# WeGoToMars/indexed_bzip2

Measured on AMD Instinct MI355X. Metric: decompressed MB/s (whole node), 2 GiB Silesia bz2-9, higher is better.
Workload: dtype u8

## Files before the change

### indexed_bzip2_amd/csrc/bz2_device.hip

```cpp
#include <hip/hip_runtime.h>

#include <cstdio>
#include <atomic>
#include <chrono>
#include <cstdlib>
#include <algorithm>
#include <cstring>
#include <condition_variable>
#include <map>
#include <memory>
#include <mutex>
#include <string>
#include <thread>
#include <vector>

#include "../../include/mi355x_bz2.h"
#include "bz2_kernels.hip.h"
#include "bz2_lines.hip.h"
#include "bz2_stage1.hip.h"
#include "bz2_hscan.hip.h"
#include "bz2_walk.hip.h"
#include "bz2_plan.hpp"
#include "bz2_scratch.hpp"
#include "bz2_lanes.hpp"
// ... 271 lines not shown
    if ( buffer.copyIssued ) {
        HIP_TRY( c, hipStreamWaitEvent( c->stream, buffer.copied, 0 ) );
    }
    if ( size + 256 > buffer.capacity ) {
        HIP_TRY( c, hipStreamSynchronize( c->stream ) );
        if ( buffer.copyIssued ) HIP_TRY( c, hipEventSynchronize( buffer.copied ) );
        HIP_TRY( c, buffer.grow( c, size + 256, size + size / 8 + ( 1u << 20 ), size ) );
    }
    buffer.copyIssued = false;
    c->outCurrent = target;
    c->dOut = buffer.bytes;
    return MI355X_BZ2_OK;
}

const char* const KERNEL_NAMES[] = {
    "(k_huff: gone)", "k_mtf<272>", "k_bwt_build", "k_walk", "k_link2", "k_emit", "k_replicate", "k_rle<false>",
    "k_rle<true>", "k_crc", "k_walk_plan", "k_mtf<144>", "k_hscan", "k_hsym"
};
constexpr uint32_t N_KERNELS = sizeof( KERNEL_NAMES ) / sizeof( KERNEL_NAMES[0] );
static_assert( N_KERNELS <= MI355X_BZ2_MAX_KERNELS );
}

struct WalkChain
{
    std::mutex mutex;
    hipEvent_t events[64]{};
    uint32_t next{ 0 };
    hipEvent_t last{ nullptr };
    std::atomic<int> liveContexts{ 0 };
};
WalkChain g_walkChains[16];
WalkChain& walkChainOf( int device ) { return g_walkChains[(unsigned)device % 16u]; }
// ... 56 lines not shown
        return v != nullptr && v[0] == '1';
    };
    BatchSwitches s;
    s.plan.scanWaves = positive( "MI355X_BZ2_SCAN_WAVES" );
    s.plan.bwtSplit = positive( "MI355X_BZ2_BWT_SPLIT" );
    s.plan.mtfNarrow = one( "MI355X_BZ2_MTF_NARROW" );
    s.plan.noSplit = one( "MI355X_BZ2_NO_SPLIT" );
    s.trace = one( "MI355X_BZ2_TRACE" );
    s.readerTrace = std::getenv( "MI355X_BZ2_READER_TRACE" ) != nullptr;
    return s;
}

int
queueOutput( mi355x_bz2_ctx* c, uint32_t n, const uint64_t* overflow )
{
    TIMED_LAUNCH( c, 0, c->stream, 8, k_rle<true>, dim3( n ), dim3( RLE_THREADS ), 0, c->stream, c->dMeta, c->dR, c->dOut,
                  overflow );
    TIMED_LAUNCH( c, 0, c->stream, 9, k_crc, dim3( n ), dim3( CRC_THREADS ), 0, c->stream, c->dMeta, c->dOut, c->crc,
                  overflow );
    HIP_TRY( c, hipEventRecord( c->evStep[2], c->stream ) );
    HIP_TRY( c, hipGetLastError() );
    HIP_TRY( c, hipMemcpyAsync( c->hMeta, c->dMeta, (size_t)n * sizeof( BlockMeta ), hipMemcpyDeviceToHost, c->stream ) );
    return MI355X_BZ2_OK;
}

int
ensureLanes( mi355x_bz2_ctx* c, const LaneLayout& layout )
{
    for ( uint32_t l = 1; l < layout.lanes; ++l ) {
        if ( (int)l == layout.highLane ) {
            if ( c->highStream == nullptr ) {
                int leastPriority = 0, greatestPriority = 0;
                (void)hipDeviceGetStreamPriorityRange( &leastPriority, &greatestPriority );
                HIP_TRY( c, hipStreamCreateWithPriority( &c->highStream, hipStreamNonBlocking, greatestPriority ) );
// ... 606 lines not shown
            const std::scoped_lock walkLock( walks.mutex );
            if ( walks.last != nullptr ) HIP_TRY( c, hipStreamWaitEvent( q, walks.last, 0 ) );
            TIMED_LAUNCH( c, g, q, 3, k_walk, walkGrid, dim3( WALK_THREADS ), 0, q,
                          meta, tab, walkPlan, walkBlk, walkPre, segLen, segSucc, plan.walkChunk, stash, segCont );
            hipEvent_t& slot = walks.events[walks.next++ % 64];
            if ( slot == nullptr ) HIP_TRY( c, hipEventCreateWithFlags( &slot, hipEventDisableTiming ) );
            HIP_TRY( c, hipEventRecord( slot, q ) );
            walks.last = slot;
        }
        TIMED_LAUNCH( c, g, q, 4, k_link2, dim3( m ), dim3( LINK_THREADS ), sizeof( LinkShared ), q, meta, segLen, segSucc, chain );
        TIMED_LAUNCH( c, g, q, 5, k_emit, dim3( ( SEG_STRIDE + EMIT_THREADS * EMIT_TILES - 1 ) / ( EMIT_THREADS * EMIT_TILES ), m ), dim3( EMIT_THREADS ), 0, q,
                      meta, tab, chain, stash, segCont, rbuf );
        static_assert( (size_t)SEG_STRIDE * STASH_BYTES >= L_STRIDE );
        TIMED_LAUNCH( c, g, q, 6, k_replicate, dim3( m ), dim3( 256 ), 0, q, meta, rbuf, reinterpret_cast<uint8_t*>( stash ),
                      (size_t)SEG_STRIDE * STASH_BYTES );
        TIMED_LAUNCH( c, g, q, 7, k_rle<false>, dim3( m ), dim3( RLE_THREADS ), 0, q, meta, rbuf, (uint8_t*)nullptr );
        lastGroupOfLane[layout.laneOf[g]] = g;
    }
    HIP_TRY( c, hipGetLastError() );
    for ( uint32_t l = 1; l < MAX_LANES; ++l ) {
        const int g = lastGroupOfLane[l];
        if ( g < 0 ) continue;
        HIP_TRY( c, hipEventRecord( c->evGroupDone[g], streamOfLane( (int)l ) ) );
        HIP_TRY( c, hipStreamWaitEvent( c->stream, c->evGroupDone[g], 0 ) );
    }

    if ( c->outputHold != nullptr ) {
        HIP_TRY( c, hipStreamWaitEvent( c->stream, c->outputHold, 0 ) );
        c->outputHold = nullptr;
    }
    hipLaunchKernelGGL( k_offsets, dim3( 1 ), dim3( OFFSETS_THREADS ), 0, c->stream, c->dMeta, c->dSlotOf, n,
                        c->out[c->outCurrent].capacity, c->dTotals );
    rc = queueOutput( c, n, c->dTotals + 1 );
    if ( rc != MI355X_BZ2_OK ) return rc;
    HIP_TRY( c, hipMemcpyAsync( c->hTotals, c->dTotals, 2 * sizeof( uint64_t ), hipMemcpyDeviceToHost, c->stream ) );
    c->pendingBlocks = n;
    if ( switches.readerTrace ) {
        const auto ms = [] ( auto a, auto b ) { return std::chrono::duration<double, std::milli>( b - a ).count(); };
        std::fprintf( stderr, "[device] begin of %u blocks: scratch %.1f ms, input %.1f ms, plan + launches %.1f ms\n", n,
                      ms( tBegin, tScratch ), ms( tScratch, tInput ), ms( tInput, std::chrono::steady_clock::now() ) );
    }
    return MI355X_BZ2_OK;
}

int
mi355x::resultBuffer( mi355x_bz2_ctx* c, uint64_t size, uint64_t keep, uint8_t** device )
{
// ... 592 lines not shown
```

### indexed_bzip2_amd/csrc/bz2_kernels.hip.h

```cpp
#pragma once

#include <hip/hip_runtime.h>
#include <stdint.h>

#include "bz2_scratch.hpp"

namespace bz2gpu
{
constexpr uint32_t MAX_N = 900000;
constexpr uint32_t MIN_SEG_STRIDE = 16;
constexpr uint32_t MARK = 0x80000000u;
constexpr uint32_t LF_MASK = 0xFFFFFu;
constexpr uint32_t INVALID_OFF = 0xFFFFFFFFu;

enum Status : int32_t {
    ST_OK = 0, ST_EOF = 1, ST_BAD_MAGIC = 2, ST_RANDOMIZED = 3, ST_ORIGPTR_RANGE = 4, ST_GROUP_COUNT = 5,
    ST_SELECTOR_COUNT = 6, ST_SELECTOR_UNARY = 7, ST_CODE_LENGTH = 8, ST_HUFFMAN_LENGTHS = 9,
    ST_SELECTOR_OVERRUN = 10, ST_INVALID_CODE = 11, ST_RUN_OVERFLOW = 12, ST_DATA_OVERFLOW = 13,
    ST_ORIGPTR_DATA = 14, ST_CRC = 15
};

struct BlockMeta
{
    uint64_t enc_off;
// ... 400 lines not shown
            R[N - 1 - k] = R[N - 1 - ( k % c )];
        }
        return;
    }
    uint8_t* const Y = tmp_buf + (size_t)b * tmp_stride;
    for ( uint32_t k = threadIdx.x; k < c; k += 256 ) Y[k] = R[N - 1 - k];
    __syncthreads();
    for ( uint32_t k = threadIdx.x; k < N; k += 256 ) {
        R[N - 1 - k] = Y[( k % c + c - r ) % c];
    }
}

constexpr uint32_t RLE_THREADS = 512;
constexpr uint32_t RLE_BYTES_PER_THREAD = 32;
constexpr uint32_t RLE_TILE = RLE_THREADS * RLE_BYTES_PER_THREAD;
constexpr uint32_t FN_IDENTITY = 0 | ( 1 << 3 ) | ( 2 << 6 ) | ( 3 << 9 ) | ( 4 << 12 );

__device__ __forceinline__ uint32_t
fn_apply( uint32_t f, uint32_t k )
{
    return ( f >> ( 3 * k ) ) & 7u;
}

__device__ __forceinline__ uint32_t
fn_compose( uint32_t f, uint32_t g )
{
    uint32_t h = 0;
#pragma unroll
    for ( int k = 0; k < 5; ++k ) h |= fn_apply( g, fn_apply( f, k ) ) << ( 3 * k );
    return h;
}

__device__ __forceinline__ uint32_t
rle_step( uint32_t k, bool eq )
{
    return eq ? ( k == 4 ? 0u : k + 1 ) : ( k == 4 ? 0u : 1u );
}

constexpr uint32_t OFFSETS_THREADS = 1024;

__global__ __launch_bounds__( OFFSETS_THREADS ) void
k_offsets( BlockMeta* meta, const uint32_t* __restrict__ slot_of, uint32_t n, uint64_t capacity, uint64_t* result )
{
    __shared__ uint64_t partial[OFFSETS_THREADS];
    const uint32_t t = threadIdx.x;
    const uint32_t per = ( n + OFFSETS_THREADS - 1 ) / OFFSETS_THREADS;
    const uint32_t lo = t * per < n ? t * per : n;
    const uint32_t hi = lo + per < n ? lo + per : n;
    uint64_t sum = 0;
    for ( uint32_t i = lo; i < hi; ++i ) {
        const BlockMeta& m = meta[slot_of[i]];
        sum += m.walk_ok ? m.decoded_size : 0;
    }
    partial[t] = sum;
    __syncthreads();
    for ( uint32_t step = 1; step < OFFSETS_THREADS; step *= 2 ) {
        const uint64_t add = t >= step ? partial[t - step] : 0;
        __syncthreads();
        partial[t] += add;
        __syncthreads();
    }
    uint64_t off = partial[t] - sum;
    for ( uint32_t i = lo; i < hi; ++i ) {
        BlockMeta& m = meta[slot_of[i]];
        m.out_off = off;
        off += m.walk_ok ? m.decoded_size : 0;
    }
    if ( t == OFFSETS_THREADS - 1 ) {
        result[0] = partial[t];
        result[1] = partial[t] + 256 > capacity ? 1 : 0;
    }
}

template<bool WRITE>
__global__ __launch_bounds__( RLE_THREADS ) void
k_rle( BlockMeta*                   meta,
       const uint8_t* __restrict__  r_buf,
       uint8_t* __restrict__        out,
       const uint64_t*              skip = nullptr )
{
    __shared__ uint32_t wfn[RLE_THREADS / 64];
    __shared__ uint64_t wsum[RLE_THREADS / 64];
    __shared__ uint32_t carryFn;
    __shared__ uint64_t carrySum;
    __shared__ uint16_t fnTab[256];
    __shared__ uint16_t cmTab[5][256];
    const uint32_t b = blockIdx.x;
    const BlockMeta mt = meta[b];
    if ( !mt.walk_ok ) return;
    if ( WRITE && skip != nullptr && *skip != 0 ) return;
    if ( threadIdx.x < 256 ) {
        const uint32_t e = threadIdx.x;
        uint32_t t[5] = { 0, 1, 2, 3, 4 };
        for ( uint32_t q = 0; q < 8; ++q ) {
            const bool eq = ( e >> q ) & 1u;
            for ( uint32_t k = 0; k < 5; ++k ) t[k] = rle_step( t[k], eq );
        }
        fnTab[e] = (uint16_t)( t[0] | ( t[1] << 3 ) | ( t[2] << 6 ) | ( t[3] << 9 ) | ( t[4] << 12 ) );
        for ( uint32_t k = 0; k < 5; ++k ) {
            uint32_t state = k, counts = 0;
            for ( uint32_t q = 0; q < 8; ++q ) {
                if ( state == 4 ) counts |= 1u << q;
                state = rle_step( state, ( e >> q ) & 1u );
            }
            cmTab[k][e] = (uint16_t)( counts | ( state << 8 ) );
        }
    }
    __syncthreads();
    const uint32_t N = mt.n;
    const uint8_t* const R = r_buf + (size_t)b * L_STRIDE;
    uint8_t* const dst = WRITE ? out + mt.out_off : nullptr;
    const uint32_t tid = threadIdx.x, wave = tid >> 6, lane = tid & 63;

    uint32_t stateIn = 0;
    uint64_t sumIn = 0;

    for ( uint32_t tile = 0; tile < N; tile += RLE_TILE ) {
        const uint32_t i0 = tile + tid * RLE_BYTES_PER_THREAD;
        uint32_t wv[RLE_BYTES_PER_THREAD / 4] = {};
        uint32_t prev = 0;
        uint32_t nb = 0;
        if ( i0 < N ) {
            nb = N - i0 < RLE_BYTES_PER_THREAD ? N - i0 : RLE_BYTES_PER_THREAD;
            const uint4 v = *reinterpret_cast<const uint4*>( R + i0 );
            const uint4 v2 = *reinterpret_cast<const uint4*>( R + i0 + 16 );
            wv[0] = v.x; wv[1] = v.y; wv[2] = v.z; wv[3] = v.w;
            wv[4] = v2.x; wv[5] = v2.y; wv[6] = v2.z; wv[7] = v2.w;
            prev = i0 > 0 ? R[i0 - 1] : 0x100u;
        }
        uint32_t eqMask = 0;
        const bool full = nb == RLE_BYTES_PER_THREAD;
        if ( full ) {
            uint32_t before = prev << 24;
#pragma unroll
            for ( uint32_t j = 0; j < RLE_BYTES_PER_THREAD / 4; ++j ) {
                const uint32_t d = wv[j] ^ __builtin_amdgcn_alignbit( wv[j], before, 24 );
                const uint32_t nonZero = ( ( ( d & 0x7F7F7F7Fu ) + 0x7F7F7F7Fu ) | d ) & 0x80808080u;
                const uint32_t e = ( ~nonZero >> 7 ) & 0x01010101u;
                eqMask |= ( ( e * 0x01020408u ) >> 24 & 0xFu ) << ( 4 * j );
                before = wv[j];
            }
            if ( prev > 0xFFu ) eqMask &= ~1u;
        } else {
            uint32_t p = prev;
            _Pragma( "unroll" ) for ( uint32_t q = 0; q < RLE_BYTES_PER_THREAD; ++q ) { if ( q >= nb ) break;
                const uint32_t c = ( wv[q >> 2] >> ( 8 * ( q & 3 ) ) ) & 0xFFu;
                eqMask |= ( c == p ? 1u : 0u ) << q;
                p = c;
            }
        }
        uint32_t fn = FN_IDENTITY;
        if ( full ) {
            fn = fn_compose( fn_compose( fnTab[eqMask & 0xFFu], fnTab[( eqMask >> 8 ) & 0xFFu] ),
                             fn_compose( fnTab[( eqMask >> 16 ) & 0xFFu], fnTab[eqMask >> 24] ) );
        } else if ( nb > 0 ) {
            uint32_t t0 = 0, t1 = 1, t2 = 2, t3 = 3, t4 = 4;
            _Pragma( "unroll" ) for ( uint32_t q = 0; q < RLE_BYTES_PER_THREAD; ++q ) { if ( q >= nb ) break;
                const bool eq = ( eqMask >> q ) & 1u;
                t0 = rle_step( t0, eq ); t1 = rle_step( t1, eq ); t2 = rle_step( t2, eq );
                t3 = rle_step( t3, eq ); t4 = rle_step( t4, eq );
            }
            fn = t0 | ( t1 << 3 ) | ( t2 << 6 ) | ( t3 << 9 ) | ( t4 << 12 );
        }
        uint32_t incl = fn;
        for ( int d = 1; d < 64; d <<= 1 ) {
            const uint32_t o = __shfl_up( incl, d );
            if ( (int)lane >= d ) incl = fn_compose( o, incl );
        }
        if ( lane == 63 ) wfn[wave] = incl;
        __syncthreads();
        uint32_t pre = FN_IDENTITY;
        for ( uint32_t w = 0; w < wave; ++w ) pre = fn_compose( pre, wfn[w] );
        uint32_t exclWave = __shfl_up( incl, 1 );
        if ( lane == 0 ) exclWave = FN_IDENTITY;
        const uint32_t before = fn_compose( pre, exclWave );
        uint32_t k = fn_apply( before, stateIn );

        uint32_t mySize = 0;
        uint32_t countMask = 0;
        if ( full ) {
            uint32_t r = cmTab[k][eqMask & 0xFFu];
            countMask = r & 0xFFu;
            r = cmTab[r >> 8][( eqMask >> 8 ) & 0xFFu];
            countMask |= ( r & 0xFFu ) << 8;
            r = cmTab[r >> 8][( eqMask >> 16 ) & 0xFFu];
            countMask |= ( r & 0xFFu ) << 16;
            r = cmTab[r >> 8][eqMask >> 24];
            countMask |= ( r & 0xFFu ) << 24;
            mySize = RLE_BYTES_PER_THREAD - (uint32_t)__popc( countMask );
            if ( countMask != 0 ) {
#pragma unroll
                for ( uint32_t j = 0; j < RLE_BYTES_PER_THREAD / 4; ++j ) {
                    const uint32_t four = ( countMask >> ( 4 * j ) ) & 0xFu;
                    if ( four != 0 ) {
#pragma unroll
                        for ( uint32_t z = 0; z < 4; ++z ) {
                            if ( ( four >> z ) & 1u ) mySize += ( wv[j] >> ( 8 * z ) ) & 0xFFu;
                        }
                    }
                }
            }
        } else {
            uint32_t kk = k;
            _Pragma( "unroll" ) for ( uint32_t q = 0; q < RLE_BYTES_PER_THREAD; ++q ) { if ( q >= nb ) break;
                const uint32_t c = ( wv[q >> 2] >> ( 8 * ( q & 3 ) ) ) & 0xFFu;
                if ( kk == 4 ) { mySize += c; countMask |= 1u << q; } else { mySize += 1; }
                kk = rle_step( kk, ( eqMask >> q ) & 1u );
            }
        }
        uint32_t inclS = mySize;
        for ( int d = 1; d < 64; d <<= 1 ) {
            const uint32_t o = __shfl_up( inclS, d );
            if ( (int)lane >= d ) inclS += o;
        }
        if ( lane == 63 ) wsum[wave] = inclS;
        __syncthreads();
        uint64_t preS = 0, tileTotal = 0;
        for ( uint32_t w = 0; w < RLE_THREADS / 64; ++w ) {
            if ( w < wave ) preS += wsum[w];
            tileTotal += wsum[w];
        }
        const uint64_t myOff = sumIn + preS + ( inclS - mySize );

        if constexpr ( WRITE ) {
            if ( countMask == 0 && nb == RLE_BYTES_PER_THREAD ) {
                uint8_t* const d = dst + myOff;
                const uint32_t head = ( 4u - ( (uint32_t)myOff & 3u ) ) & 3u;
                for ( uint32_t z = 0; z < head; ++z ) d[z] = (uint8_t)( wv[0] >> ( 8 * z ) );
                uint32_t* const d32 = reinterpret_cast<uint32_t*>( d + head );
#pragma unroll
                for ( uint32_t j = 0; j + 1 < RLE_BYTES_PER_THREAD / 4; ++j ) {
                    d32[j] = __builtin_amdgcn_alignbyte( wv[j + 1], wv[j], head );
                }
                constexpr uint32_t LAST = RLE_BYTES_PER_THREAD / 4 - 1;
                if ( head == 0 ) {
                    d32[LAST] = wv[LAST];
                } else {
                    for ( uint32_t z = head; z < 4; ++z ) d[4 * LAST + z] = (uint8_t)( wv[LAST] >> ( 8 * z ) );
                }
            } else {
            uint64_t o = myOff;
            uint32_t p = prev;
            _Pragma( "unroll" ) for ( uint32_t q = 0; q < RLE_BYTES_PER_THREAD; ++q ) { if ( q >= nb ) break;
                const uint32_t c = ( wv[q >> 2] >> ( 8 * ( q & 3 ) ) ) & 0xFFu;
                if ( ( countMask >> q ) & 1u ) {
                    for ( uint32_t z = 0; z < c; ++z ) dst[o + z] = (uint8_t)p;
                    o += c;
                } else {
                    dst[o++] = (uint8_t)c;
                }
                p = c;
            }
            }
        }

        if ( tid == RLE_THREADS - 1 ) {
            carryFn = fn_apply( fn_compose( before, fn ), stateIn );
        }
        __syncthreads();
        stateIn = carryFn;
        sumIn += tileTotal;
        __syncthreads();
    }
    if ( !WRITE && tid == 0 ) {
        meta[b].decoded_size = sumIn;
    }
    (void)carrySum;
}

constexpr uint32_t CRC_THREADS = 256;
constexpr uint32_t CRC_CHUNK_LOG2 = 8;
constexpr uint32_t CRC_CHUNK = 1u << CRC_CHUNK_LOG2;
constexpr uint32_t CRC_TILE = CRC_THREADS * CRC_CHUNK;
constexpr uint32_t CRC_POLY = 0x04C11DB7u;

__device__ __forceinline__ uint32_t
gf_mul( uint32_t a, uint32_t b )
{
    uint32_t r = 0;
#pragma unroll 8
    for ( int i = 31; i >= 0; --i ) {
        r = ( r << 1 ) ^ ( ( r >> 31 ) ? CRC_POLY : 0u );
        if ( ( a >> i ) & 1u ) r ^= b;
    }
    return r;
}

__device__ __forceinline__ uint32_t
gf_pow8( const uint32_t* table, uint64_t nbytes )
{
    uint32_t r = 0x00000001u;
    for ( int k = 0; nbytes != 0 && k < 32; ++k, nbytes >>= 1 ) {
        if ( nbytes & 1u ) r = gf_mul( r, table[k] );
    }
    return r;
}

__global__ __launch_bounds__( CRC_THREADS ) void
k_crc( BlockMeta*                  meta,
       const uint8_t* __restrict__ out,
       CrcConsts                   cc,
       const uint64_t*             skip = nullptr )
{
    __shared__ uint32_t table[256];
    __shared__ uint32_t wcrc[CRC_THREADS / 64];
    const uint32_t b = blockIdx.x;
// ... 56 lines not shown
            running = gf_mul( running, cc.pow8[CRC_CHUNK_LOG2 + 8] ) ^ tileCrc;
        }
        __syncthreads();
        tEnd = t + CRC_TILE;
    }
    if ( tid == 0 ) {
        const uint64_t pad = tEnd - a1;
        uint32_t pure = D == 0 ? 0u : gf_mul( running, gf_pow8( cc.ipow8, pad ) );
        const uint32_t init = gf_mul( 0xFFFFFFFFu, gf_pow8( cc.pow8, D ) );
        const uint32_t crc = ~( pure ^ init );
        meta[b].computed_crc = crc;
        if ( crc != mt.header_crc ) meta[b].status = ST_CRC;
    }
}

constexpr uint32_t GATHER_THREADS = 256;
constexpr uint64_t GATHER_TILE = 32768;

struct GatherTile
{
    uint64_t src, dst, size;
};

__global__ __launch_bounds__( GATHER_THREADS ) void
k_gather( const GatherTile* __restrict__ tiles, const uint8_t* __restrict__ src, uint8_t* __restrict__ dst )
{
    const GatherTile t = tiles[blockIdx.x];
    const uint8_t* const s = src + t.src;
    uint8_t* const d = dst + t.dst;
    const uint32_t n = (uint32_t)t.size;
// ... 32 lines not shown
```

### indexed_bzip2_amd/csrc/bz2_scratch.hpp

```cpp
#pragma once

#include <algorithm>
#include <cstdint>

#include "bz2_plan.hpp"

namespace bz2gpu
{
constexpr uint32_t L_STRIDE = 900096;
constexpr uint32_t SEL_STRIDE = 32768;
constexpr uint32_t TAB_STRIDE = 1u << 20;
constexpr uint32_t KMAX = 32768;
constexpr uint32_t SEG_STRIDE = KMAX + 64;
constexpr uint32_t STASH_BYTES = 128;
constexpr uint32_t SYM_STRIDE = SEG_STRIDE * 64;
constexpr uint32_t GPOS_STRIDE = 18048;
constexpr int BWT_WAVES = 16;
constexpr uint32_t BWT_COUNTS_PER_BLOCK = BWT_SPLIT_MAX * BWT_WAVES * 256;

struct ScratchSizes
{
    uint64_t blockMeta, huffMeta, scanMeta, huffTables, walkPlan;
};

enum ScratchMemory : bool { DEVICE = false, PINNED = true };

#define BZ2_SCRATCH_REGIONS( X )                                                                                              \
    X( DEVICE, dOffsets, uint64_t, n * sizeof( uint64_t ), OWN )                                                              \
    X( DEVICE, dOrder, uint32_t, n * sizeof( uint32_t ), OWN )                                                                \
    X( DEVICE, dMeta, BlockMeta, n * s.blockMeta, OWN )                                                                       \
    X( DEVICE, dSel, uint8_t, n * SEL_STRIDE + 256, OWN )                                                                     \
    X( DEVICE, dStb, uint8_t, n * 256, OWN )                                                                                  \
    X( DEVICE, dHmeta, HuffMeta, n * s.huffMeta, OWN )                                                                        \
    X( DEVICE, dSmeta, ScanMeta, n * s.scanMeta, OWN )                                                 \
    X( DEVICE, dHtab, HuffTables, n * s.huffTables, OWN )                                        \
    X( DEVICE, dGpos, uint32_t, n * GPOS_STRIDE * sizeof( uint32_t ), OWN )                                                   \
    X( DEVICE, dL, uint8_t, n * L_STRIDE + 256, OWN )                                                                         \
    X( DEVICE, dTab, uint32_t, n * TAB_STRIDE * sizeof( uint32_t ), OWN )                                                     \
        \
    X( DEVICE, dR, uint8_t, n * L_STRIDE + 256, keepStages ? OWN : R_dL )                                                     \
    X( DEVICE, dSegLen, uint32_t, n * SEG_STRIDE * sizeof( uint32_t ), OWN )                                                  \
    X( DEVICE, dSegSucc, uint32_t, n * SEG_STRIDE * sizeof( uint32_t ), OWN )                                                 \
    X( DEVICE, dSegCont, uint32_t, n * SEG_STRIDE * sizeof( uint32_t ), OWN )  \
    X( DEVICE, dChain, uint2, n * SEG_STRIDE * 2 * sizeof( uint32_t ), OWN )  \
    X( DEVICE, dStash, uint32_t, n * SEG_STRIDE * STASH_BYTES, OWN )                        \
        \
    X( DEVICE, dSym, uint16_t, n * SYM_STRIDE * sizeof( uint16_t ), R_dStash )                                                \
    X( DEVICE, dPlan, WalkPlan, MAX_GROUPS * s.walkPlan, OWN )                                             \
    X( DEVICE, dWalkBlk, uint32_t, MAX_GROUPS * ( n + 16 ) * sizeof( uint32_t ), OWN )                                        \
    X( DEVICE, dWalkPre, uint32_t, MAX_GROUPS * ( n + 16 ) * sizeof( uint32_t ), OWN )                                        \
    X( DEVICE, dSlotOf, uint32_t, n * sizeof( uint32_t ), OWN )                                                               \
    X( DEVICE, dTotals, uint64_t, 2 * sizeof( uint64_t ), OWN )           \
    X( DEVICE, dBwtCounts, uint32_t, std::min<size_t>( n, BWT_SPLIT_BLOCKS ) * BWT_COUNTS_PER_BLOCK * sizeof( uint32_t ), OWN )  \
    X( DEVICE, dEnds, uint64_t, n * sizeof( uint64_t ), OWN )                        \
    X( PINNED, hOrder, uint32_t, n * sizeof( uint32_t ), OWN )                                                                \
    X( PINNED, hSlotOf, uint32_t, n * sizeof( uint32_t ), OWN )                                   \
// ... 54 lines not shown
```

Before: 34670.

## Split RLE sizing and expansion into per-block pieces with CRC folding

Each block's final RLE decode used to run as one workgroup. It is now split into RLE_PIECES workgroups per block. A sizing pass records, for every piece, its state transition and its size for each possible entry state. k_offsets then chains the pieces to find each piece's entry state and output offset. The expand kernel writes each piece and computes a partial CRC, and a new k_crc_fold kernel combines those partials with GF(2) shifts, replacing the separate k_crc pass over the output. This raises parallelism per block and drops one full read of the output, at the cost of more kernel complexity, computing sizes for five entry states when the entry state is unknown, and reusing segSucc scratch to hold the piece records.

```diff
diff --git a/indexed_bzip2_amd/csrc/bz2_device.hip b/indexed_bzip2_amd/csrc/bz2_device.hip
--- a/indexed_bzip2_amd/csrc/bz2_device.hip
+++ b/indexed_bzip2_amd/csrc/bz2_device.hip
@@ -309,8 +309,8 @@
 }
 
 const char* const KERNEL_NAMES[] = {
-    "(k_huff: gone)", "k_mtf<272>", "k_bwt_build", "k_walk", "k_link2", "k_emit", "k_replicate", "k_rle<false>",
-    "k_rle<true>", "k_crc", "k_walk_plan", "k_mtf<144>", "k_hscan", "k_hsym"
+    "(k_huff: gone)", "k_mtf<272>", "k_bwt_build", "k_walk", "k_link2", "k_emit", "k_replicate", "k_rle_size",
+    "k_rle_expand", "k_crc_fold", "k_walk_plan", "k_mtf<144>", "k_hscan", "k_hsym"
 };
 constexpr uint32_t N_KERNELS = sizeof( KERNEL_NAMES ) / sizeof( KERNEL_NAMES[0] );
 static_assert( N_KERNELS <= MI355X_BZ2_MAX_KERNELS );
@@ -397,10 +397,9 @@
 int
 queueOutput( mi355x_bz2_ctx* c, uint32_t n, const uint64_t* overflow )
 {
-    TIMED_LAUNCH( c, 0, c->stream, 8, k_rle<true>, dim3( n ), dim3( RLE_THREADS ), 0, c->stream, c->dMeta, c->dR, c->dOut,
-                  overflow );
-    TIMED_LAUNCH( c, 0, c->stream, 9, k_crc, dim3( n ), dim3( CRC_THREADS ), 0, c->stream, c->dMeta, c->dOut, c->crc,
-                  overflow );
+    TIMED_LAUNCH( c, 0, c->stream, 8, k_rle_expand, dim3( RLE_PIECES, n ), dim3( RLE_THREADS ), 0, c->stream, c->dMeta, c->dR,
+                  c->dOut, c->dSegSucc, c->crc, overflow );
+    TIMED_LAUNCH( c, 0, c->stream, 9, k_crc_fold, dim3( n ), dim3( 64 ), 0, c->stream, c->dMeta, c->dSegSucc, c->crc, overflow );
     HIP_TRY( c, hipEventRecord( c->evStep[2], c->stream ) );
     HIP_TRY( c, hipGetLastError() );
     HIP_TRY( c, hipMemcpyAsync( c->hMeta, c->dMeta, (size_t)n * sizeof( BlockMeta ), hipMemcpyDeviceToHost, c->stream ) );
@@ -1037,7 +1036,7 @@
         static_assert( (size_t)SEG_STRIDE * STASH_BYTES >= L_STRIDE );
         TIMED_LAUNCH( c, g, q, 6, k_replicate, dim3( m ), dim3( 256 ), 0, q, meta, rbuf, reinterpret_cast<uint8_t*>( stash ),
                       (size_t)SEG_STRIDE * STASH_BYTES );
-        TIMED_LAUNCH( c, g, q, 7, k_rle<false>, dim3( m ), dim3( RLE_THREADS ), 0, q, meta, rbuf, (uint8_t*)nullptr );
+        TIMED_LAUNCH( c, g, q, 7, k_rle_size, dim3( RLE_PIECES, m ), dim3( RLE_THREADS ), 0, q, meta, rbuf, segSucc );
         lastGroupOfLane[layout.laneOf[g]] = g;
     }
     HIP_TRY( c, hipGetLastError() );
@@ -1053,7 +1052,7 @@
         c->outputHold = nullptr;
     }
     hipLaunchKernelGGL( k_offsets, dim3( 1 ), dim3( OFFSETS_THREADS ), 0, c->stream, c->dMeta, c->dSlotOf, n,
-                        c->out[c->outCurrent].capacity, c->dTotals );
+                        c->out[c->outCurrent].capacity, c->dTotals, c->dSegSucc );
     rc = queueOutput( c, n, c->dTotals + 1 );
     if ( rc != MI355X_BZ2_OK ) return rc;
     HIP_TRY( c, hipMemcpyAsync( c->hTotals, c->dTotals, 2 * sizeof( uint64_t ), hipMemcpyDeviceToHost, c->stream ) );
diff --git a/indexed_bzip2_amd/csrc/bz2_kernels.hip.h b/indexed_bzip2_amd/csrc/bz2_kernels.hip.h
--- a/indexed_bzip2_amd/csrc/bz2_kernels.hip.h
+++ b/indexed_bzip2_amd/csrc/bz2_kernels.hip.h
@@ -438,6 +438,7 @@
 constexpr uint32_t RLE_THREADS = 512;
 constexpr uint32_t RLE_BYTES_PER_THREAD = 32;
 constexpr uint32_t RLE_TILE = RLE_THREADS * RLE_BYTES_PER_THREAD;
+constexpr uint32_t RLE_WAVES = RLE_THREADS / 64;
 constexpr uint32_t FN_IDENTITY = 0 | ( 1 << 3 ) | ( 2 << 6 ) | ( 3 << 9 ) | ( 4 << 12 );
 
 __device__ __forceinline__ uint32_t
@@ -455,16 +456,272 @@
     return h;
 }
 
-__device__ __forceinline__ uint32_t
+__device__ __forceinline__ bool
+fn_is_const( uint32_t f )
+{
+    return f == ( f & 7u ) * 0x1249u;
+}
+
+__host__ __device__ constexpr uint32_t
 rle_step( uint32_t k, bool eq )
 {
     return eq ? ( k == 4 ? 0u : k + 1 ) : ( k == 4 ? 0u : 1u );
 }
 
+__device__ __forceinline__ uint32_t
+rle_piece_tiles( uint32_t n )
+{
+    const uint32_t tiles = ( n + RLE_TILE - 1 ) / RLE_TILE;
+    return ( tiles + RLE_PIECES - 1 ) / RLE_PIECES;
+}
+
+struct RleTables
+{
+    uint16_t fn[256];
+    uint16_t cm[5][256];
+};
+
+constexpr RleTables
+makeRleTables()
+{
+    RleTables r{};
+    for ( uint32_t e = 0; e < 256; ++e ) {
+        uint32_t t[5] = { 0, 1, 2, 3, 4 };
+        for ( uint32_t q = 0; q < 8; ++q ) {
+            for ( uint32_t k = 0; k < 5; ++k ) t[k] = rle_step( t[k], ( e >> q ) & 1u );
+        }
+        r.fn[e] = (uint16_t)( t[0] | ( t[1] << 3 ) | ( t[2] << 6 ) | ( t[3] << 9 ) | ( t[4] << 12 ) );
+        for ( uint32_t k = 0; k < 5; ++k ) {
+            uint32_t state = k, counts = 0;
+            for ( uint32_t q = 0; q < 8; ++q ) {
+                if ( state == 4 ) counts |= 1u << q;
+                state = rle_step( state, ( e >> q ) & 1u );
+            }
+            r.cm[k][e] = (uint16_t)( counts | ( state << 8 ) );
+        }
+    }
+    return r;
+}
+
+__device__ const RleTables RLE_TABLES = makeRleTables();
+
+__device__ __forceinline__ void
+rle_load_tables( RleTables& lds )
+{
+    static_assert( sizeof( RleTables ) % 4 == 0 );
+    const auto* const from = reinterpret_cast<const uint32_t*>( &RLE_TABLES );
+    auto* const to = reinterpret_cast<uint32_t*>( &lds );
+    for ( uint32_t i = threadIdx.x; i < sizeof( RleTables ) / 4; i += RLE_THREADS ) to[i] = from[i];
+}
+
+using RleBytes = uint32_t[RLE_BYTES_PER_THREAD / 4];
+
+struct RleChunk
+{
+    uint32_t prev;
+    uint32_t nb;
+    uint32_t eqMask;
+    uint32_t fn;
+};
+
+__device__ __forceinline__ uint32_t
+rle_byte( const RleBytes& wv, uint32_t q )
+{
+    return ( wv[q >> 2] >> ( 8 * ( q & 3 ) ) ) & 0xFFu;
+}
+
+__device__ __forceinline__ void
+rle_load_chunk( RleBytes& wv, RleChunk& c, const uint8_t* __restrict__ R, uint32_t N, uint32_t i0, const RleTables& tab )
+{
+#pragma unroll
+    for ( uint32_t j = 0; j < RLE_BYTES_PER_THREAD / 4; ++j ) wv[j] = 0;
+    c.prev = 0;
+    c.nb = 0;
+    if ( i0 < N ) {
+        c.nb = N - i0 < RLE_BYTES_PER_THREAD ? N - i0 : RLE_BYTES_PER_THREAD;
+        const uint4 v = *reinterpret_cast<const uint4*>( R + i0 );
+        const uint4 v2 = *reinterpret_cast<const uint4*>( R + i0 + 16 );
+        wv[0] = v.x; wv[1] = v.y; wv[2] = v.z; wv[3] = v.w;
+        wv[4] = v2.x; wv[5] = v2.y; wv[6] = v2.z; wv[7] = v2.w;
+        c.prev = i0 > 0 ? R[i0 - 1] : 0x100u;
+    }
+    c.eqMask = 0;
+    c.fn = FN_IDENTITY;
+    if ( c.nb == RLE_BYTES_PER_THREAD ) {
+        uint32_t before = c.prev << 24;
+#pragma unroll
+        for ( uint32_t j = 0; j < RLE_BYTES_PER_THREAD / 4; ++j ) {
+            const uint32_t d = wv[j] ^ __builtin_amdgcn_alignbit( wv[j], before, 24 );
+            const uint32_t nonZero = ( ( ( d & 0x7F7F7F7Fu ) + 0x7F7F7F7Fu ) | d ) & 0x80808080u;
+            const uint32_t e = ( ~nonZero >> 7 ) & 0x01010101u;
+            c.eqMask |= ( ( e * 0x01020408u ) >> 24 & 0xFu ) << ( 4 * j );
+            before = wv[j];
+        }
+        if ( c.prev > 0xFFu ) c.eqMask &= ~1u;
+        c.fn = fn_compose( fn_compose( tab.fn[c.eqMask & 0xFFu], tab.fn[( c.eqMask >> 8 ) & 0xFFu] ),
+                           fn_compose( tab.fn[( c.eqMask >> 16 ) & 0xFFu], tab.fn[c.eqMask >> 24] ) );
+    } else if ( c.nb > 0 ) {
+        const uint32_t nb = c.nb;
+        uint32_t p = c.prev, eqMask = 0;
+        _Pragma( "unroll" ) for ( uint32_t q = 0; q < RLE_BYTES_PER_THREAD; ++q ) { if ( q >= nb ) break;
+            const uint32_t b = rle_byte( wv, q );
+            eqMask |= ( b == p ? 1u : 0u ) << q;
+            p = b;
+        }
+        uint32_t t0 = 0, t1 = 1, t2 = 2, t3 = 3, t4 = 4;
+        _Pragma( "unroll" ) for ( uint32_t q = 0; q < RLE_BYTES_PER_THREAD; ++q ) { if ( q >= nb ) break;
+            const bool eq = ( eqMask >> q ) & 1u;
+            t0 = rle_step( t0, eq ); t1 = rle_step( t1, eq ); t2 = rle_step( t2, eq );
+            t3 = rle_step( t3, eq ); t4 = rle_step( t4, eq );
+        }
+        c.eqMask = eqMask;
+        c.fn = t0 | ( t1 << 3 ) | ( t2 << 6 ) | ( t3 << 9 ) | ( t4 << 12 );
+    }
+}
+
+__device__ __forceinline__ uint32_t
+rle_chunk_size( const RleBytes& wv, const RleChunk& c, uint32_t k, const RleTables& tab, uint32_t& countMask )
+{
+    uint32_t size = 0;
+    countMask = 0;
+    if ( c.nb == RLE_BYTES_PER_THREAD ) {
+        uint32_t r = tab.cm[k][c.eqMask & 0xFFu];
+        countMask = r & 0xFFu;
+        r = tab.cm[r >> 8][( c.eqMask >> 8 ) & 0xFFu];
+        countMask |= ( r & 0xFFu ) << 8;
+        r = tab.cm[r >> 8][( c.eqMask >> 16 ) & 0xFFu];
+        countMask |= ( r & 0xFFu ) << 16;
+        r = tab.cm[r >> 8][c.eqMask >> 24];
+        countMask |= ( r & 0xFFu ) << 24;
+        size = RLE_BYTES_PER_THREAD - (uint32_t)__popc( countMask );
+        if ( countMask != 0 ) {
+#pragma unroll
+            for ( uint32_t j = 0; j < RLE_BYTES_PER_THREAD / 4; ++j ) {
+                const uint32_t four = ( countMask >> ( 4 * j ) ) & 0xFu;
+                if ( four != 0 ) {
+#pragma unroll
+                    for ( uint32_t z = 0; z < 4; ++z ) {
+                        if ( ( four >> z ) & 1u ) size += ( wv[j] >> ( 8 * z ) ) & 0xFFu;
+                    }
+                }
+            }
+        }
+    } else {
+        const uint32_t nb = c.nb, eqMask = c.eqMask;
+        uint32_t counts = 0;
+        _Pragma( "unroll" ) for ( uint32_t q = 0; q < RLE_BYTES_PER_THREAD; ++q ) { if ( q >= nb ) break;
+            if ( k == 4 ) { size += rle_byte( wv, q ); counts |= 1u << q; } else { size += 1; }
+            k = rle_step( k, ( eqMask >> q ) & 1u );
+        }
+        countMask = counts;
+    }
+    return size;
+}
+
+__device__ __forceinline__ uint32_t
+rle_wave_scan( uint32_t fn, uint32_t lane, uint32_t& total )
+{
+    uint32_t incl = fn;
+    if ( __ballot( !fn_is_const( fn ) ) != 0 ) {
+        for ( int d = 1; d < 64; d <<= 1 ) {
+            const uint32_t o = __shfl_up( incl, d );
+            if ( (int)lane >= d && !fn_is_const( incl ) ) incl = fn_compose( o, incl );
+        }
+    }
+    uint32_t excl = __shfl_up( incl, 1 );
+    if ( lane == 0 ) excl = FN_IDENTITY;
+    total = __shfl( incl, 63 );
+    return excl;
+}
+
+__device__ __forceinline__ uint32_t
+wave_sum( uint32_t v )
+{
+    for ( int d = 32; d > 0; d >>= 1 ) v += __shfl_xor( v, d );
+    return v;
+}
+
+__global__ __launch_bounds__( RLE_THREADS ) void
+k_rle_size( const BlockMeta* __restrict__ meta, const uint8_t* __restrict__ r_buf, uint32_t* seg_succ )
+{
+    __shared__ RleTables tab;
+    __shared__ uint32_t wfn[2][RLE_WAVES];
+    __shared__ uint32_t wacc[6][RLE_WAVES];
+    const uint32_t b = blockIdx.y, piece = blockIdx.x;
+    const BlockMeta& mt = meta[b];
+    if ( !mt.walk_ok ) return;
+    const uint32_t N = mt.n;
+    const uint32_t perPiece = rle_piece_tiles( N );
+    const uint32_t begin = piece * perPiece * RLE_TILE;
+    const uint32_t end = min( N, ( piece + 1 ) * perPiece * RLE_TILE );
+    RlePiece& record = rlePieces( seg_succ, b )[piece];
+    if ( begin >= end ) {
+        if ( threadIdx.x == 0 ) {
+            record.fn = FN_IDENTITY;
+            for ( uint32_t j = 0; j < 5; ++j ) record.size[j] = 0;
+        }
+        return;
+    }
+    rle_load_tables( tab );
+    __syncthreads();
+    const uint8_t* const R = r_buf + (size_t)b * L_STRIDE;
+    const uint32_t tid = threadIdx.x, wave = sfl( tid >> 6 ), lane = tid & 63;
+
+    uint32_t carry = FN_IDENTITY;
+    uint32_t accAll = 0;
+    uint32_t acc[5] = {};
+    uint32_t parity = 0;
+    for ( uint32_t tile = begin; tile < end; tile += RLE_TILE, parity ^= 1u ) {
+        RleBytes wv;
+        RleChunk c;
+        rle_load_chunk( wv, c, R, N, tile + tid * RLE_BYTES_PER_THREAD, tab );
+        uint32_t waveFn;
+        const uint32_t excl = rle_wave_scan( c.fn, lane, waveFn );
+        if ( lane == 0 ) wfn[parity][wave] = waveFn;
+        __syncthreads();
+        uint32_t pre = FN_IDENTITY, tileFn = FN_IDENTITY;
+        for ( uint32_t w = 0; w < RLE_WAVES; ++w ) {
+            if ( w == wave ) pre = tileFn;
+            const uint32_t g = sfl( wfn[parity][w] );
+            tileFn = fn_is_const( g ) ? g : fn_compose( tileFn, g );
+        }
+        const uint32_t toWave = fn_is_const( pre ) ? pre : fn_compose( carry, pre );
+        const uint32_t before = lane == 0 ? toWave : ( fn_is_const( excl ) ? excl : fn_compose( toWave, excl ) );
+        uint32_t countMask;
+        if ( __ballot( !fn_is_const( before ) ) == 0 ) {
+            accAll += rle_chunk_size( wv, c, before & 7u, tab, countMask );
+        } else {
+#pragma unroll
+            for ( uint32_t j = 0; j < 5; ++j ) acc[j] += rle_chunk_size( wv, c, fn_apply( before, j ), tab, countMask );
+        }
+        carry = fn_is_const( tileFn ) ? tileFn : fn_compose( carry, tileFn );
+    }
+    accAll = wave_sum( accAll );
+#pragma unroll
+    for ( uint32_t j = 0; j < 5; ++j ) acc[j] = wave_sum( acc[j] );
+    if ( lane == 0 ) {
+        wacc[5][wave] = accAll;
+#pragma unroll
+        for ( uint32_t j = 0; j < 5; ++j ) wacc[j][wave] = acc[j];
+    }
+    __syncthreads();
+    if ( tid == 0 ) {
+        uint32_t all = 0;
+        for ( uint32_t w = 0; w < RLE_WAVES; ++w ) all += wacc[5][w];
+        for ( uint32_t j = 0; j < 5; ++j ) {
+            uint32_t s = all;
+            for ( uint32_t w = 0; w < RLE_WAVES; ++w ) s += wacc[j][w];
+            record.size[j] = s;
+        }
+        record.fn = carry;
+    }
+}
+
 constexpr uint32_t OFFSETS_THREADS = 1024;
 
 __global__ __launch_bounds__( OFFSETS_THREADS ) void
-k_offsets( BlockMeta* meta, const uint32_t* __restrict__ slot_of, uint32_t n, uint64_t capacity, uint64_t* result )
+k_offsets( BlockMeta* meta, const uint32_t* __restrict__ slot_of, uint32_t n, uint64_t capacity, uint64_t* result,
+           uint32_t* seg_succ )
 {
     __shared__ uint64_t partial[OFFSETS_THREADS];
     const uint32_t t = threadIdx.x;
@@ -473,8 +730,20 @@
     const uint32_t hi = lo + per < n ? lo + per : n;
     uint64_t sum = 0;
     for ( uint32_t i = lo; i < hi; ++i ) {
-        const BlockMeta& m = meta[slot_of[i]];
-        sum += m.walk_ok ? m.decoded_size : 0;
+        const uint32_t slot = slot_of[i];
+        BlockMeta& m = meta[slot];
+        if ( !m.walk_ok ) continue;
+        RlePiece* const pieces = rlePieces( seg_succ, slot );
+        uint32_t state = 0;
+        uint64_t bytes = 0;
+        for ( uint32_t p = 0; p < RLE_PIECES; ++p ) {
+            pieces[p].entry = state;
+            pieces[p].offset = bytes;
+            bytes += pieces[p].size[state];
+            state = fn_apply( pieces[p].fn, state );
+        }
+        m.decoded_size = bytes;
+        sum += bytes;
     }
     partial[t] = sum;
     __syncthreads();
@@ -496,209 +765,13 @@
     }
 }
 
-template<bool WRITE>
-__global__ __launch_bounds__( RLE_THREADS ) void
-k_rle( BlockMeta*                   meta,
-       const uint8_t* __restrict__  r_buf,
-       uint8_t* __restrict__        out,
-       const uint64_t*              skip = nullptr )
-{
-    __shared__ uint32_t wfn[RLE_THREADS / 64];
-    __shared__ uint64_t wsum[RLE_THREADS / 64];
-    __shared__ uint32_t carryFn;
-    __shared__ uint64_t carrySum;
-    __shared__ uint16_t fnTab[256];
-    __shared__ uint16_t cmTab[5][256];
-    const uint32_t b = blockIdx.x;
-    const BlockMeta mt = meta[b];
-    if ( !mt.walk_ok ) return;
-    if ( WRITE && skip != nullptr && *skip != 0 ) return;
-    if ( threadIdx.x < 256 ) {
-        const uint32_t e = threadIdx.x;
-        uint32_t t[5] = { 0, 1, 2, 3, 4 };
-        for ( uint32_t q = 0; q < 8; ++q ) {
-            const bool eq = ( e >> q ) & 1u;
-            for ( uint32_t k = 0; k < 5; ++k ) t[k] = rle_step( t[k], eq );
-        }
-        fnTab[e] = (uint16_t)( t[0] | ( t[1] << 3 ) | ( t[2] << 6 ) | ( t[3] << 9 ) | ( t[4] << 12 ) );
-        for ( uint32_t k = 0; k < 5; ++k ) {
-            uint32_t state = k, counts = 0;
-            for ( uint32_t q = 0; q < 8; ++q ) {
-                if ( state == 4 ) counts |= 1u << q;
-                state = rle_step( state, ( e >> q ) & 1u );
-            }
-            cmTab[k][e] = (uint16_t)( counts | ( state << 8 ) );
-        }
-    }
-    __syncthreads();
-    const uint32_t N = mt.n;
-    const uint8_t* const R = r_buf + (size_t)b * L_STRIDE;
-    uint8_t* const dst = WRITE ? out + mt.out_off : nullptr;
-    const uint32_t tid = threadIdx.x, wave = tid >> 6, lane = tid & 63;
-
-    uint32_t stateIn = 0;
-    uint64_t sumIn = 0;
-
-    for ( uint32_t tile = 0; tile < N; tile += RLE_TILE ) {
-        const uint32_t i0 = tile + tid * RLE_BYTES_PER_THREAD;
-        uint32_t wv[RLE_BYTES_PER_THREAD / 4] = {};
-        uint32_t prev = 0;
-        uint32_t nb = 0;
-        if ( i0 < N ) {
-            nb = N - i0 < RLE_BYTES_PER_THREAD ? N - i0 : RLE_BYTES_PER_THREAD;
-            const uint4 v = *reinterpret_cast<const uint4*>( R + i0 );
-            const uint4 v2 = *reinterpret_cast<const uint4*>( R + i0 + 16 );
-            wv[0] = v.x; wv[1] = v.y; wv[2] = v.z; wv[3] = v.w;
-            wv[4] = v2.x; wv[5] = v2.y; wv[6] = v2.z; wv[7] = v2.w;
-            prev = i0 > 0 ? R[i0 - 1] : 0x100u;
-        }
-        uint32_t eqMask = 0;
-        const bool full = nb == RLE_BYTES_PER_THREAD;
-        if ( full ) {
-            uint32_t before = prev << 24;
-#pragma unroll
-            for ( uint32_t j = 0; j < RLE_BYTES_PER_THREAD / 4; ++j ) {
-                const uint32_t d = wv[j] ^ __builtin_amdgcn_alignbit( wv[j], before, 24 );
-                const uint32_t nonZero = ( ( ( d & 0x7F7F7F7Fu ) + 0x7F7F7F7Fu ) | d ) & 0x80808080u;
-                const uint32_t e = ( ~nonZero >> 7 ) & 0x01010101u;
-                eqMask |= ( ( e * 0x01020408u ) >> 24 & 0xFu ) << ( 4 * j );
-                before = wv[j];
-            }
-            if ( prev > 0xFFu ) eqMask &= ~1u;
-        } else {
-            uint32_t p = prev;
-            _Pragma( "unroll" ) for ( uint32_t q = 0; q < RLE_BYTES_PER_THREAD; ++q ) { if ( q >= nb ) break;
-                const uint32_t c = ( wv[q >> 2] >> ( 8 * ( q & 3 ) ) ) & 0xFFu;
-                eqMask |= ( c == p ? 1u : 0u ) << q;
-                p = c;
-            }
-        }
-        uint32_t fn = FN_IDENTITY;
-        if ( full ) {
-            fn = fn_compose( fn_compose( fnTab[eqMask & 0xFFu], fnTab[( eqMask >> 8 ) & 0xFFu] ),
-                             fn_compose( fnTab[( eqMask >> 16 ) & 0xFFu], fnTab[eqMask >> 24] ) );
-        } else if ( nb > 0 ) {
-            uint32_t t0 = 0, t1 = 1, t2 = 2, t3 = 3, t4 = 4;
-            _Pragma( "unroll" ) for ( uint32_t q = 0; q < RLE_BYTES_PER_THREAD; ++q ) { if ( q >= nb ) break;
-                const bool eq = ( eqMask >> q ) & 1u;
-                t0 = rle_step( t0, eq ); t1 = rle_step( t1, eq ); t2 = rle_step( t2, eq );
-                t3 = rle_step( t3, eq ); t4 = rle_step( t4, eq );
-            }
-            fn = t0 | ( t1 << 3 ) | ( t2 << 6 ) | ( t3 << 9 ) | ( t4 << 12 );
-        }
-        uint32_t incl = fn;
-        for ( int d = 1; d < 64; d <<= 1 ) {
-            const uint32_t o = __shfl_up( incl, d );
-            if ( (int)lane >= d ) incl = fn_compose( o, incl );
-        }
-        if ( lane == 63 ) wfn[wave] = incl;
-        __syncthreads();
-        uint32_t pre = FN_IDENTITY;
-        for ( uint32_t w = 0; w < wave; ++w ) pre = fn_compose( pre, wfn[w] );
-        uint32_t exclWave = __shfl_up( incl, 1 );
-        if ( lane == 0 ) exclWave = FN_IDENTITY;
-        const uint32_t before = fn_compose( pre, exclWave );
-        uint32_t k = fn_apply( before, stateIn );
-
-        uint32_t mySize = 0;
-        uint32_t countMask = 0;
-        if ( full ) {
-            uint32_t r = cmTab[k][eqMask & 0xFFu];
-            countMask = r & 0xFFu;
-            r = cmTab[r >> 8][( eqMask >> 8 ) & 0xFFu];
-            countMask |= ( r & 0xFFu ) << 8;
-            r = cmTab[r >> 8][( eqMask >> 16 ) & 0xFFu];
-            countMask |= ( r & 0xFFu ) << 16;
-            r = cmTab[r >> 8][eqMask >> 24];
-            countMask |= ( r & 0xFFu ) << 24;
-            mySize = RLE_BYTES_PER_THREAD - (uint32_t)__popc( countMask );
-            if ( countMask != 0 ) {
-#pragma unroll
-                for ( uint32_t j = 0; j < RLE_BYTES_PER_THREAD / 4; ++j ) {
-                    const uint32_t four = ( countMask >> ( 4 * j ) ) & 0xFu;
-                    if ( four != 0 ) {
-#pragma unroll
-                        for ( uint32_t z = 0; z < 4; ++z ) {
-                            if ( ( four >> z ) & 1u ) mySize += ( wv[j] >> ( 8 * z ) ) & 0xFFu;
-                        }
-                    }
-                }
-            }
-        } else {
-            uint32_t kk = k;
-            _Pragma( "unroll" ) for ( uint32_t q = 0; q < RLE_BYTES_PER_THREAD; ++q ) { if ( q >= nb ) break;
-                const uint32_t c = ( wv[q >> 2] >> ( 8 * ( q & 3 ) ) ) & 0xFFu;
-                if ( kk == 4 ) { mySize += c; countMask |= 1u << q; } else { mySize += 1; }
-                kk = rle_step( kk, ( eqMask >> q ) & 1u );
-            }
-        }
-        uint32_t inclS = mySize;
-        for ( int d = 1; d < 64; d <<= 1 ) {
-            const uint32_t o = __shfl_up( inclS, d );
-            if ( (int)lane >= d ) inclS += o;
-        }
-        if ( lane == 63 ) wsum[wave] = inclS;
-        __syncthreads();
-        uint64_t preS = 0, tileTotal = 0;
-        for ( uint32_t w = 0; w < RLE_THREADS / 64; ++w ) {
-            if ( w < wave ) preS += wsum[w];
-            tileTotal += wsum[w];
-        }
-        const uint64_t myOff = sumIn + preS + ( inclS - mySize );
-
-        if constexpr ( WRITE ) {
-            if ( countMask == 0 && nb == RLE_BYTES_PER_THREAD ) {
-                uint8_t* const d = dst + myOff;
-                const uint32_t head = ( 4u - ( (uint32_t)myOff & 3u ) ) & 3u;
-                for ( uint32_t z = 0; z < head; ++z ) d[z] = (uint8_t)( wv[0] >> ( 8 * z ) );
-                uint32_t* const d32 = reinterpret_cast<uint32_t*>( d + head );
-#pragma unroll
-                for ( uint32_t j = 0; j + 1 < RLE_BYTES_PER_THREAD / 4; ++j ) {
-                    d32[j] = __builtin_amdgcn_alignbyte( wv[j + 1], wv[j], head );
-                }
-                constexpr uint32_t LAST = RLE_BYTES_PER_THREAD / 4 - 1;
-                if ( head == 0 ) {
-                    d32[LAST] = wv[LAST];
-                } else {
-                    for ( uint32_t z = head; z < 4; ++z ) d[4 * LAST + z] = (uint8_t)( wv[LAST] >> ( 8 * z ) );
-                }
-            } else {
-            uint64_t o = myOff;
-            uint32_t p = prev;
-            _Pragma( "unroll" ) for ( uint32_t q = 0; q < RLE_BYTES_PER_THREAD; ++q ) { if ( q >= nb ) break;
-                const uint32_t c = ( wv[q >> 2] >> ( 8 * ( q & 3 ) ) ) & 0xFFu;
-                if ( ( countMask >> q ) & 1u ) {
-                    for ( uint32_t z = 0; z < c; ++z ) dst[o + z] = (uint8_t)p;
-                    o += c;
-                } else {
-                    dst[o++] = (uint8_t)c;
-                }
-                p = c;
-            }
-            }
-        }
-
-        if ( tid == RLE_THREADS - 1 ) {
-            carryFn = fn_apply( fn_compose( before, fn ), stateIn );
-        }
-        __syncthreads();
-        stateIn = carryFn;
-        sumIn += tileTotal;
-        __syncthreads();
-    }
-    if ( !WRITE && tid == 0 ) {
-        meta[b].decoded_size = sumIn;
-    }
-    (void)carrySum;
-}
-
 constexpr uint32_t CRC_THREADS = 256;
 constexpr uint32_t CRC_CHUNK_LOG2 = 8;
 constexpr uint32_t CRC_CHUNK = 1u << CRC_CHUNK_LOG2;
 constexpr uint32_t CRC_TILE = CRC_THREADS * CRC_CHUNK;
 constexpr uint32_t CRC_POLY = 0x04C11DB7u;
 
-__device__ __forceinline__ uint32_t
+__host__ __device__ constexpr uint32_t
 gf_mul( uint32_t a, uint32_t b )
 {
     uint32_t r = 0;
@@ -714,6 +787,7 @@
 gf_pow8( const uint32_t* table, uint64_t nbytes )
 {
     uint32_t r = 0x00000001u;
+#pragma nounroll
     for ( int k = 0; nbytes != 0 && k < 32; ++k, nbytes >>= 1 ) {
         if ( nbytes & 1u ) r = gf_mul( r, table[k] );
     }
@@ -800,6 +874,240 @@
     }
 }
 
+struct CrcTables
+{
+    uint32_t byte[256];
+    uint32_t behind[RLE_THREADS];
+    uint32_t lo[256], hi[256];
+};
+
+constexpr CrcTables
+makeCrcTables()
+{
+    CrcTables t{};
+    for ( uint32_t i = 0; i < 256; ++i ) {
+        uint32_t c = i << 24;
+        for ( int j = 0; j < 8; ++j ) c = ( c & 0x80000000u ) ? ( c << 1 ) ^ CRC_POLY : ( c << 1 );
+        t.byte[i] = c;
+    }
+    uint32_t chunk = 0x100u;
+    for ( uint32_t bytes = 1; bytes < RLE_BYTES_PER_THREAD; bytes *= 2 ) chunk = gf_mul( chunk, chunk );
+    uint32_t p = 1u;
+    for ( uint32_t lane = RLE_THREADS; lane-- > 0; ) {
+        t.behind[lane] = p;
+        p = gf_mul( p, chunk );
+    }
+    uint32_t x256 = 0x100u;
+    for ( uint32_t bytes = 1; bytes < 256; bytes *= 2 ) x256 = gf_mul( x256, x256 );
+    uint32_t l = 1u, h = 1u;
+    for ( uint32_t j = 0; j < 256; ++j ) {
+        t.lo[j] = l;
+        t.hi[j] = h;
+        l = gf_mul( l, 0x100u );
+        h = gf_mul( h, x256 );
+    }
+    return t;
+}
+
+__device__ const CrcTables CRC_TABLES = makeCrcTables();
+
+__device__ __forceinline__ uint32_t
+wave_xor( uint32_t v )
+{
+    for ( int d = 32; d > 0; d >>= 1 ) v ^= __shfl_xor( v, d );
+    return v;
+}
+
+struct CrcShared
+{
+    uint32_t byte[256], lo[256], hi[256];
+};
+
+__device__ __forceinline__ uint32_t
+crc_shift( const CrcShared& t, const CrcConsts& cc, uint32_t n )
+{
+    uint32_t r = gf_mul( t.lo[n & 0xFFu], t.hi[( n >> 8 ) & 0xFFu] );
+    if ( ( n >> 16 ) != 0 ) r = gf_mul( r, gf_pow8( cc.pow8 + 16, n >> 16 ) );
+    return r;
+}
+
+__global__ __launch_bounds__( RLE_THREADS ) void
+k_rle_expand( const BlockMeta* __restrict__ meta,
+              const uint8_t* __restrict__   r_buf,
+              uint8_t* __restrict__         out,
+              uint32_t*                     seg_succ,
+              CrcConsts                     cc,
+              const uint64_t*               skip )
+{
+    __shared__ RleTables tab;
+    __shared__ CrcShared crcTab;
+    __shared__ uint32_t wfn[RLE_WAVES];
+    __shared__ uint32_t wsum[RLE_WAVES];
+    __shared__ uint32_t wcrc[2][RLE_WAVES];
+    constexpr uint32_t KEEPS = 0x80000000u;
+    const uint32_t b = blockIdx.y, piece = blockIdx.x;
+    const BlockMeta& mt = meta[b];
+    if ( !mt.walk_ok ) return;
+    if ( skip != nullptr && *skip != 0 ) return;
+    const uint32_t N = mt.n;
+    const uint32_t perPiece = rle_piece_tiles( N );
+    const uint32_t begin = piece * perPiece * RLE_TILE;
+    const uint32_t end = min( N, ( piece + 1 ) * perPiece * RLE_TILE );
+    RlePiece& record = rlePieces( seg_succ, b )[piece];
+    if ( begin >= end ) {
+        if ( threadIdx.x == 0 ) {
+            record.crc = 0;
+            record.bytes = 0;
+        }
+        return;
+    }
+    rle_load_tables( tab );
+    if ( threadIdx.x < 256 ) {
+        crcTab.byte[threadIdx.x] = CRC_TABLES.byte[threadIdx.x];
+        crcTab.lo[threadIdx.x] = CRC_TABLES.lo[threadIdx.x];
+        crcTab.hi[threadIdx.x] = CRC_TABLES.hi[threadIdx.x];
+    }
+    __syncthreads();
+    const uint8_t* const R = r_buf + (size_t)b * L_STRIDE;
+    uint8_t* const dst = out + mt.out_off + record.offset;
+    const uint32_t tid = threadIdx.x, wave = sfl( tid >> 6 ), lane = tid & 63;
+    const uint32_t behindFull = CRC_TABLES.behind[tid];
+
+    uint32_t stateIn = sfl( record.entry );
+    uint64_t sumIn = 0;
+    uint32_t running = 0;
+    uint32_t lastTotal = 0;
+    bool lastKeeps = false;
+    const auto foldLastTile = [&] ( uint32_t parity ) {
+        uint32_t tileCrc = 0;
+        for ( uint32_t w = 0; w < RLE_WAVES; ++w ) tileCrc ^= wcrc[parity][w];
+        running = gf_mul( running, lastKeeps ? cc.pow8[14] : crc_shift( crcTab, cc, lastTotal ) ) ^ tileCrc;
+    };
+    static_assert( RLE_TILE == 1u << 14 );
+
+    uint32_t parity = 0;
+    for ( uint32_t tile = begin; tile < end; tile += RLE_TILE, parity ^= 1u ) {
+        RleBytes wv;
+        RleChunk c;
+        rle_load_chunk( wv, c, R, N, tile + tid * RLE_BYTES_PER_THREAD, tab );
+        uint32_t waveFn;
+        const uint32_t excl = rle_wave_scan( c.fn, lane, waveFn );
+        if ( lane == 0 ) wfn[wave] = waveFn;
+        __syncthreads();
+        if ( wave == 0 && tile != begin ) foldLastTile( parity ^ 1u );
+        uint32_t state = stateIn, stateWave = stateIn;
+        for ( uint32_t w = 0; w < RLE_WAVES; ++w ) {
+            if ( w == wave ) stateWave = state;
+            state = fn_apply( sfl( wfn[w] ), state );
+        }
+        uint32_t countMask;
+        const uint32_t mySize = rle_chunk_size( wv, c, fn_apply( excl, stateWave ), tab, countMask );
+        uint32_t inclS = mySize;
+        for ( int d = 1; d < 64; d <<= 1 ) {
+            const uint32_t o = __shfl_up( inclS, d );
+            if ( (int)lane >= d ) inclS += o;
+        }
+        const bool waveKeeps = __ballot( mySize != RLE_BYTES_PER_THREAD ) == 0;
+        if ( lane == 63 ) wsum[wave] = inclS | ( waveKeeps ? KEEPS : 0u );
+        __syncthreads();
+        uint32_t preS = 0, tileTotal = 0;
+        bool keeps = true;
+        for ( uint32_t w = 0; w < RLE_WAVES; ++w ) {
+            const uint32_t s = sfl( wsum[w] );
+            if ( w < wave ) preS += s & ~KEEPS;
+            tileTotal += s & ~KEEPS;
+            keeps = keeps && ( s & KEEPS ) != 0;
+        }
+        const uint32_t inTile = preS + inclS - mySize;
+        const uint64_t myOff = sumIn + inTile;
+
+        uint32_t crc = 0;
+        const auto crcByte = [&] ( uint32_t byte ) { crc = ( crc << 8 ) ^ crcTab.byte[( crc >> 24 ) ^ byte]; };
+        if ( countMask == 0 && c.nb == RLE_BYTES_PER_THREAD ) {
+            uint8_t* const d = dst + myOff;
+            const uint32_t head = ( 4u - ( (uint32_t)reinterpret_cast<uintptr_t>( d ) & 3u ) ) & 3u;
+            for ( uint32_t z = 0; z < head; ++z ) d[z] = (uint8_t)( wv[0] >> ( 8 * z ) );
+            uint32_t* const d32 = reinterpret_cast<uint32_t*>( d + head );
+#pragma unroll
+            for ( uint32_t j = 0; j + 1 < RLE_BYTES_PER_THREAD / 4; ++j ) {
+                d32[j] = __builtin_amdgcn_alignbyte( wv[j + 1], wv[j], head );
+            }
+            constexpr uint32_t LAST = RLE_BYTES_PER_THREAD / 4 - 1;
+            if ( head == 0 ) {
+                d32[LAST] = wv[LAST];
+            } else {
+                for ( uint32_t z = head; z < 4; ++z ) d[4 * LAST + z] = (uint8_t)( wv[LAST] >> ( 8 * z ) );
+            }
+#pragma unroll
+            for ( uint32_t q = 0; q < RLE_BYTES_PER_THREAD; ++q ) crcByte( rle_byte( wv, q ) );
+        } else {
+            const uint32_t nb = c.nb;
+            uint64_t o = myOff;
+            uint32_t p = c.prev;
+            _Pragma( "unroll" ) for ( uint32_t q = 0; q < RLE_BYTES_PER_THREAD; ++q ) { if ( q >= nb ) break;
+                const uint32_t v = rle_byte( wv, q );
+                if ( ( countMask >> q ) & 1u ) {
+                    for ( uint32_t z = 0; z < v; ++z ) {
+                        dst[o + z] = (uint8_t)p;
+                        crcByte( p );
+                    }
+                    o += v;
+                } else {
+                    dst[o++] = (uint8_t)v;
+                    crcByte( v );
+                }
+                p = v;
+            }
+        }
+        uint32_t term;
+        if ( keeps ) {
+            term = gf_mul( crc, behindFull );
+        } else {
+            term = gf_mul( crc, crc_shift( crcTab, cc, tileTotal - inTile - mySize ) );
+        }
+        term = wave_xor( term );
+        if ( lane == 0 ) wcrc[parity][wave] = term;
+
+        lastTotal = tileTotal;
+        lastKeeps = keeps;
+        stateIn = state;
+        sumIn += tileTotal;
+    }
+    __syncthreads();
+    if ( wave == 0 ) {
+        foldLastTile( parity ^ 1u );
+        if ( tid == 0 ) {
+            record.crc = running;
+            record.bytes = sumIn;
+        }
+    }
+}
+
+static_assert( RLE_PIECES < 64 );
+
+__global__ __launch_bounds__( 64 ) void
+k_crc_fold( BlockMeta* meta, uint32_t* seg_succ, CrcConsts cc, const uint64_t* skip )
+{
+    const uint32_t b = blockIdx.x;
+    const BlockMeta& mt = meta[b];
+    if ( !mt.walk_ok ) return;
+    if ( skip != nullptr && *skip != 0 ) return;
+    const uint32_t lane = threadIdx.x;
+    const uint64_t D = mt.decoded_size;
+    uint32_t term = 0;
+    if ( lane < RLE_PIECES ) {
+        const RlePiece& p = rlePieces( seg_succ, b )[lane];
+        term = gf_mul( p.crc, gf_pow8( cc.pow8, D - p.offset - p.bytes ) );
+    } else if ( lane == RLE_PIECES ) {
+        term = gf_mul( 0xFFFFFFFFu, gf_pow8( cc.pow8, D ) );
+    }
+    const uint32_t crc = ~wave_xor( term );
+    if ( lane == 0 ) {
+        meta[b].computed_crc = crc;
+        if ( crc != mt.header_crc ) meta[b].status = ST_CRC;
+    }
+}
+
 constexpr uint32_t GATHER_THREADS = 256;
 constexpr uint64_t GATHER_TILE = 32768;
 
diff --git a/indexed_bzip2_amd/csrc/bz2_scratch.hpp b/indexed_bzip2_amd/csrc/bz2_scratch.hpp
--- a/indexed_bzip2_amd/csrc/bz2_scratch.hpp
+++ b/indexed_bzip2_amd/csrc/bz2_scratch.hpp
@@ -17,6 +17,34 @@
 constexpr uint32_t GPOS_STRIDE = 18048;
 constexpr int BWT_WAVES = 16;
 constexpr uint32_t BWT_COUNTS_PER_BLOCK = BWT_SPLIT_MAX * BWT_WAVES * 256;
+
+constexpr uint32_t RLE_PIECES = 8;
+
+struct RlePiece
+{
+    uint32_t fn;
+    uint32_t size[5];
+    uint32_t entry;
+    uint32_t crc;
+    uint64_t offset;
+    uint64_t bytes;
+};
+
+static_assert( sizeof( RlePiece ) == 48 );
+static_assert( RLE_PIECES * sizeof( RlePiece ) <= SEG_STRIDE * sizeof( uint32_t ) );
+static_assert( SEG_STRIDE * sizeof( uint32_t ) % alignof( RlePiece ) == 0 );
+
+#if defined( __HIPCC__ )
+#define BZ2_HOST_DEVICE __host__ __device__
+#else
+#define BZ2_HOST_DEVICE
+#endif
+
+BZ2_HOST_DEVICE inline RlePiece*
+rlePieces( uint32_t* segSucc, uint32_t block )
+{
+    return reinterpret_cast<RlePiece*>( segSucc + (size_t)block * SEG_STRIDE );
+}
 
 struct ScratchSizes
 {
@@ -40,6 +68,7 @@
         \
     X( DEVICE, dR, uint8_t, n * L_STRIDE + 256, keepStages ? OWN : R_dL )                                                     \
     X( DEVICE, dSegLen, uint32_t, n * SEG_STRIDE * sizeof( uint32_t ), OWN )                                                  \
+        \
     X( DEVICE, dSegSucc, uint32_t, n * SEG_STRIDE * sizeof( uint32_t ), OWN )                                                 \
     X( DEVICE, dSegCont, uint32_t, n * SEG_STRIDE * sizeof( uint32_t ), OWN )  \
     X( DEVICE, dChain, uint2, n * SEG_STRIDE * 2 * sizeof( uint32_t ), OWN )  \
```

Result: slower. 34150 (-1.5%).
